# shamspias/fennec

Hardware: AMD Instinct MI355X
Metric: megapixels/sec: 4K SSIMFast+GaussianBlur (higher is better)
Workload: dtype u8 (blur: exact int32 sums of 24-bit fixed-point weights on the i8 matrix pipe; fp64 SSIM)

## Files before the change

fennec_amd/csrc/blur_mfma.hip:

```cpp
#include <hip/hip_ext.h>

#include "common.hpp"
#include "devutil.hpp"

#include <algorithm>
#include <cmath>
#include <type_traits>
#include <vector>

namespace fnx {

typedef int v4i __attribute__((ext_vector_type(4)));

constexpr int MF_RMAX = 6;
constexpr int MF_P = 48;
constexpr int MF_WT = 64 * MF_P + 256;
constexpr int MF_SP = 352;
constexpr int MF_OP = 272;
constexpr int MF_SEG_SCORE = 272;
constexpr int MF_SEG_SCORE_WIDE = 544;

struct MfmaArgs {
    const uint8_t *src;
    const uint8_t *const *srcs;
    uint8_t *dst;
    uint8_t *const *dsts;
    int sstride, dstride, w, h;
    int tiles_x, tiles, seg;
    int radius;
    const uint32_t *tab;
    int seed_h, seed_v, thr;
    const int32_t *bx, *by;
    const uint32_t *coltab, *rowtab;
    unsigned long long *slabs;
    int nbx, nby;
    int dbg;
    int narrow;
};

__device__ __forceinline__ int mf_comb3(int hi, int mid, int lo)
{
    int t = hi * 256 + mid;
    asm volatile("" : "+v"(t));
    return t * 256 + lo;
}

__device__ __forceinline__ const double *mf_scalar_ptr(const double *p)
{
    const unsigned long long v = reinterpret_cast<unsigned long long>(p);
    const unsigned lo = __builtin_amdgcn_readfirstlane(static_cast<unsigned>(v)), hi = __builtin_amdgcn_readfirstlane(static_cast<unsigned>(v >> 32));
    return reinterpret_cast<const double *>((static_cast<unsigned long long>(hi) << 32) | lo);
}
typedef __attribute__((address_space(1))) uint8_t mf_g_u8;
template <typename T> __device__ __forceinline__ T *mf_sgpr_ptr(T *p)
{
    unsigned long long v = reinterpret_cast<unsigned long long>(p);
    asm volatile("" : "+s"(v));
    return reinterpret_cast<T *>(v);
}
__device__ __forceinline__ void mf_lane_off(uint32_t &o) { asm volatile("" : "+v"(o)); }
typedef int mf_s16i __attribute__((ext_vector_type(16)));
__device__ __forceinline__ uint32_t mf_exact_u(const double *wd, const uint8_t *base, int step, int ring0, int mask)
{
    mf_s16i w0, w1;
    asm volatile("s_load_dwordx16 %0, %2, 0x0\n\ts_load_dwordx16 %1, %2, 0x40\n\ts_waitcnt lgkmcnt(0)" : "=&s"(w0), "=&s"(w1) : "s"(mf_scalar_ptr(wd)) : "memory");
    uint32_t v[13];
#pragma unroll
    for (int t = 0; t < 13; t++) v[t] = base[((ring0 + t) & mask) * step];
    double acc = 0;
#pragma unroll
    for (int t = 0; t < 13; t++) {
        const int lo = t < 8 ? w0[2 * (t & 7)] : w1[2 * (t & 7)], hi = t < 8 ? w0[2 * (t & 7) + 1] : w1[2 * (t & 7) + 1];
        acc = acc + u8_to_f64(v[t] ^ 0x80u) * __hiloint2double(hi, lo);
    }
    return clampF_dev(acc);
}

__device__ __forceinline__ void mf_box_add4(uint32_t *tbl, const u32x4 ro, uint32_t coln, const v4i cb)
{
#pragma unroll
    for (int k = 0; k < 4; k++)
        __hip_atomic_fetch_add(reinterpret_cast<uint32_t *>(reinterpret_cast<char *>(tbl) + ro[k] + coln), static_cast<uint32_t>(cb[k]),
                               __ATOMIC_RELAXED, __HIP_MEMORY_SCOPE_WORKGROUP);
}

template <bool SCORE, bool GUARD>
__global__ __launch_bounds__(256, GUARD ? 3 : 1) void blur_mfma_kernel(MfmaArgs a)
{
    constexpr int P = MF_P, WT = MF_WT, SP = MF_SP, OP = MF_OP;
    __shared__ __attribute__((aligned(16))) uint8_t s_t[4 * WT];
    __shared__ __attribute__((aligned(16))) uint8_t s_stage[2 * 16 * SP];
    __shared__ __attribute__((aligned(16))) uint8_t s_out[2 * 16 * OP];
    __shared__ __attribute__((aligned(16))) uint32_t s_rowh[SCORE ? MF_SEG_SCORE + 32 : 4];
    __shared__ __attribute__((aligned(16))) uint32_t s_rowv[SCORE ? MF_SEG_SCORE + 16 : 4];
    extern __shared__ __attribute__((aligned(16))) uint32_t s_box[];

    const int tile = xcd_tile(blockIdx.x, a.tiles);
    if (tile < 0) return;
    const int z = blockIdx.y;
    const uint8_t *src = a.srcs ? a.srcs[z] : a.src;
    uint8_t *dst = a.dsts ? a.dsts[z] : a.dst;
    const int ty = tile / a.tiles_x, tx = tile - ty * a.tiles_x;
    const int x0 = tx * 64, y0 = ty * a.seg;
    const int tid = threadIdx.x, wave = tid >> 6, lane = tid & 63;
    const int r = lane & 15, g = lane >> 4;
    const int NJ = min(a.seg, ((a.h - y0 + 15) >> 4) << 4) >> 4;
    const int NI = NJ + 1;
    const bool xedge = x0 - 6 < 0 || x0 + 70 > a.w;

    const v4i *tbh = reinterpret_cast<const v4i *>(a.tab);
    const long *tbv = reinterpret_cast<const long *>(a.tab + 3 * 64 * 4);
    const v4i bh2 = tbh[lane], bh1 = tbh[64 + lane], bh0 = tbh[128 + lane];
    const long bv2 = tbv[lane], bv1 = tbv[64 + lane], bv0 = tbv[128 + lane];
    const bool alane = (r & 3) == 3;
    const int seed_hl = alane ? (1 << 23) + 128 : a.seed_h;
    const v4i sh = {seed_hl, seed_hl, seed_hl, seed_hl}, sv = {a.seed_v, a.seed_v, a.seed_v, a.seed_v};
    const v4i zero = {0, 0, 0, 0};
    const uint32_t sel01 = alane ? 0x0c0c0400u : 0x0c0c0703u, sel23 = alane ? 0x04000c0cu : 0x07030c0cu;

    uint8_t *tw = s_t + wave * WT;
    const int id1 = min(256 + tid, 16 * 19 - 1);
    const int srow0 = tid / 19, sch0 = tid - 19 * srow0, srow1 = id1 / 19, sch1 = id1 - 19 * srow1;
    const bool two = tid < 48;
    const int st_w0 = srow0 * SP + 16 * sch0, st_w1 = srow1 * SP + 16 * sch1;
    const int st_r = r * SP + 64 * wave + 16 * g;
    uint8_t *t_w = tw + r * P + 4 * g;
    const int m4 = r >> 2, mi = r & 3;
    const uint8_t *t_r = tw + (16 * m4 + mi) * P + 64 * m4 + 8 * g;
    const uint8_t *t_ro = tw + (16 * m4 + mi) * P + 64 * m4 + ((8 * g + 16) & 31);
    const uint8_t *t_ae = tw + (16 * g + 3) * P + 64 * g + r + 6;
    const uint8_t *t_ao = tw + (16 * g + 3) * P + 64 * g + ((r + 22) & 31);
    const int o_w = r * OP + 64 * wave + 16 * g;
    const int orow = tid >> 4, och = tid & 15;
    const int o_r = orow * OP + 16 * och;
    const int xo = x0 + 4 * och;

    v4i bbox = {0, 0, 0, 0}, sbox = {0, 0, 0, 0};
    uint32_t coln = 0;
    const int slabn = SCORE ? (a.nbx + 1) * (a.nby + 1) : 0;
    uint32_t *tbl_s = s_box, *tbl_b = s_box + 4 * slabn;
    auto score_setup = [&]() {
        const uint32_t cw = a.coltab[256 * tx + tid];
        const int nrow = (2 * a.seg + 16) >> 2;
        const int nrh = (a.seg + 16) >> 2;
        const u32x4 rw = reinterpret_cast<const u32x4 *>(a.rowtab)[static_cast<size_t>(ty) * nrow + min(tid, nrow - 1)];
        if (!(a.dbg & 4)) for (int e = tid; e < 2 * slabn; e += 256) reinterpret_cast<u32x4 *>(s_box)[e] = (u32x4){0u, 0u, 0u, 0u};
        if (tid < nrh) reinterpret_cast<u32x4 *>(s_rowh)[tid] = rw;
        else if (tid < nrow) reinterpret_cast<u32x4 *>(s_rowv)[tid - nrh] = rw;
        coln = cw & 0xfffffu;
        const int seed = static_cast<int>((cw >> 20) & 31u) << 7;
        sbox = (v4i){seed, seed, seed, seed};
        const uint32_t sh = (cw >> 29) << 3;
#pragma unroll
        for (int e = 0; e < 4; e++) bbox[e] = static_cast<int>(((cw >> (25 + e)) & 1u) << sh);
    };

    const double *wd = reinterpret_cast<const double *>(a.tab + 3 * 64 * 4 + 3 * 64 * 2);

    auto stage_write = [&](const u32x4 (&d)[2], int buf) {
        uint8_t *sb = s_stage + buf * 16 * SP;
        *reinterpret_cast<u32x4 *>(sb + st_w0) = d[0] ^ 0x80808080u;
        if (two) *reinterpret_cast<u32x4 *>(sb + st_w1) = d[1] ^ 0x80808080u;
    };
    auto hset = [&](int s, int buf, int slot) {
        const uint8_t *sbuf = s_stage + buf * 16 * SP;
        const uint8_t *sb = sbuf + st_r;
        if constexpr (!GUARD && !SCORE) {
#pragma unroll
            for (int hf = 0; hf < 2; hf++) {
                v4i c2[2], c1[2], c0[2];
#pragma unroll
                for (int q2 = 0; q2 < 2; q2++) {
                    const v4i A = *reinterpret_cast<const v4i *>(sb + 16 * (2 * hf + q2));
                    c2[q2] = __builtin_amdgcn_mfma_i32_16x16x64_i8(A, bh2, zero, 0, 0, 0);
                    c1[q2] = __builtin_amdgcn_mfma_i32_16x16x64_i8(A, bh1, zero, 0, 0, 0);
                    c0[q2] = __builtin_amdgcn_mfma_i32_16x16x64_i8(A, bh0, sh, 0, 0, 0);
                }
#pragma unroll
                for (int q2 = 0; q2 < 2; q2++) {
                    const int qq = 2 * hf + q2;
                    v4i u;
#pragma unroll
                    for (int k = 0; k < 4; k++) u[k] = mf_comb3(c2[q2][k], c1[q2][k], c0[q2][k]);
                    const uint32_t t01 = __builtin_amdgcn_perm((uint32_t)u[1], (uint32_t)u[0], sel01);
                    const uint32_t t23 = __builtin_amdgcn_perm((uint32_t)u[3], (uint32_t)u[2], sel23);
                    *reinterpret_cast<uint32_t *>(t_w + (16 * qq) * P + 64 * qq + 16 * slot) = t01 | t23;
                }
                __builtin_amdgcn_sched_barrier(0);
            }
            return;
        }
        v4i c2[4], c1[4], c0[4];
#pragma unroll
        for (int qq = 0; qq < 4; qq++) {
            const v4i A = *reinterpret_cast<const v4i *>(sb + 16 * qq);
            c2[qq] = __builtin_amdgcn_mfma_i32_16x16x64_i8(A, bh2, zero, 0, 0, 0);
            c1[qq] = __builtin_amdgcn_mfma_i32_16x16x64_i8(A, bh1, zero, 0, 0, 0);
            c0[qq] = __builtin_amdgcn_mfma_i32_16x16x64_i8(A, bh0, sh, 0, 0, 0);
        }
        if constexpr (SCORE) {
            const u32x2 lo = *reinterpret_cast<const u32x2 *>(sb + 24), hi = *reinterpret_cast<const u32x2 *>(sb + 32);
            const v4i A = {(int)lo.x, (int)lo.y, (int)hi.x, (int)hi.y};
            const v4i cb = __builtin_amdgcn_mfma_i32_16x16x64_i8(A, bbox, sbox, 0, 0, 0);
            const u32x4 ro = *reinterpret_cast<const u32x4 *>(s_rowh + 16 * s + 4 * g);
            if (!(a.dbg & 1)) mf_box_add4(tbl_s, ro, coln, cb);
        }
        v4i u[4];
#pragma unroll
        for (int qq = 0; qq < 4; qq++)
#pragma unroll
            for (int k = 0; k < 4; k++) u[qq][k] = mf_comb3(c2[qq][k], c1[qq][k], c0[qq][k]);
#pragma unroll
        for (int qq = 0; qq < 4; qq++) {
            const uint32_t t01 = __builtin_amdgcn_perm((uint32_t)u[qq][1], (uint32_t)u[qq][0], sel01);
            const uint32_t t23 = __builtin_amdgcn_perm((uint32_t)u[qq][3], (uint32_t)u[qq][2], sel23);
            *reinterpret_cast<uint32_t *>(t_w + (16 * qq) * P + 64 * qq + 16 * slot) = t01 | t23;
        }
        if constexpr (GUARD) {
            uint32_t m[4];
#pragma unroll
            for (int qq = 0; qq < 4; qq++) {
                const uint32_t f0 = static_cast<uint32_t>(u[qq][0]) & 0x00ffffffu, f1 = static_cast<uint32_t>(u[qq][1]) & 0x00ffffffu;
                const uint32_t f2 = static_cast<uint32_t>(u[qq][2]) & 0x00ffffffu, f3 = static_cast<uint32_t>(u[qq][3]) & 0x00ffffffu;
                m[qq] = min(min(min(f0, f1), f2), f3);
            }
            const uint32_t mm = min(min(min(m[0], m[1]), m[2]), m[3]);
            if (__builtin_amdgcn_ballot_w64(mm < static_cast<uint32_t>(a.thr))) {
                uint32_t fl = 0;
#pragma unroll
                for (int qq = 0; qq < 4; qq++)
#pragma unroll
                    for (int k = 0; k < 4; k++) fl |= ((static_cast<uint32_t>(u[qq][k]) & 0x00ffffffu) < static_cast<uint32_t>(a.thr) ? 1u : 0u) << (4 * qq + k);
                unsigned long long todo = __builtin_amdgcn_ballot_w64(fl != 0);
                while (todo) {
                    const int L = __builtin_ctzll(todo);
                    todo &= todo - 1;
                    uint32_t flL = __builtin_amdgcn_readlane(fl, L);
                    const int rL = L & 15, gL = L >> 4;
                    while (flL) {
                        const int b = __builtin_ctz(flL), qq = b >> 2, k = b & 3;
                        flL &= flL - 1;
                        const uint32_t e = mf_exact_u(wd, sbuf + (4 * gL + k) * SP + 4 * (16 * wave + 4 * qq + (rL >> 2)) + (rL & 3), 4, 0, 0xffff) ^ 0x80u;
                        if (lane == L) *(t_w + (16 * qq) * P + 64 * qq + 16 * slot + k) = static_cast<uint8_t>(e);
                    }
                }
            }
        }
    };
    auto vset = [&](int j, int buf, auto oddt) {
        constexpr bool ODD = decltype(oddt)::value;
        long A[4];
        uint32_t al[4];
#pragma unroll
        for (int q = 0; q < 4; q++) A[q] = *reinterpret_cast<const long *>((ODD ? t_ro : t_r) + (4 * q) * P);
#pragma unroll
        for (int q = 0; q < 4; q++) al[q] = *((ODD ? t_ao : t_ae) + (4 * q) * P);
        int u[4][3];
        if constexpr (!GUARD && !SCORE) {
#pragma unroll
            for (int hf = 0; hf < 2; hf++) {
                v4i c2[2], c1[2], c0[2];
#pragma unroll
                for (int q2 = 0; q2 < 2; q2++) {
                    c2[q2] = __builtin_amdgcn_mfma_i32_16x16x32_i8(A[2 * hf + q2], bv2, zero, 0, 0, 0);
                    c1[q2] = __builtin_amdgcn_mfma_i32_16x16x32_i8(A[2 * hf + q2], bv1, zero, 0, 0, 0);
                    c0[q2] = __builtin_amdgcn_mfma_i32_16x16x32_i8(A[2 * hf + q2], bv0, sv, 0, 0, 0);
                }
#pragma unroll
                for (int q2 = 0; q2 < 2; q2++)
#pragma unroll
                    for (int i = 0; i < 3; i++) u[2 * hf + q2][i] = mf_comb3(c2[q2][i], c1[q2][i], c0[q2][i]);
                __builtin_amdgcn_sched_barrier(0);
            }
        } else {
            v4i c2[4], c1[4], c0[4];
#pragma unroll
            for (int q = 0; q < 4; q++) {
                c2[q] = __builtin_amdgcn_mfma_i32_16x16x32_i8(A[q], bv2, zero, 0, 0, 0);
                c1[q] = __builtin_amdgcn_mfma_i32_16x16x32_i8(A[q], bv1, zero, 0, 0, 0);
                c0[q] = __builtin_amdgcn_mfma_i32_16x16x32_i8(A[q], bv0, sv, 0, 0, 0);
            }
#pragma unroll
            for (int q = 0; q < 4; q++)
#pragma unroll
                for (int i = 0; i < 3; i++) u[q][i] = mf_comb3(c2[q][i], c1[q][i], c0[q][i]);
        }
        u32x4 o;
#pragma unroll
        for (int q = 0; q < 4; q++) {
            const uint32_t t01 = __builtin_amdgcn_perm((uint32_t)u[q][1], (uint32_t)u[q][0], 0x0c0c0703u);
            const uint32_t t23 = __builtin_amdgcn_perm(al[q], (uint32_t)u[q][2], 0x04030c0cu);
            o[q] = t01 | t23;
        }
        uint8_t *op = s_out + buf * 16 * OP + o_w;
        *reinterpret_cast<u32x4 *>(op) = o;
        if constexpr (GUARD) {
            uint32_t m[4];
#pragma unroll
            for (int q = 0; q < 4; q++)
                m[q] = min(min(static_cast<uint32_t>(u[q][0]) & 0x00ffffffu, static_cast<uint32_t>(u[q][1]) & 0x00ffffffu), static_cast<uint32_t>(u[q][2]) & 0x00ffffffu);
            const uint32_t mm = min(min(min(m[0], m[1]), m[2]), m[3]);
            if (__builtin_amdgcn_ballot_w64(mm < static_cast<uint32_t>(a.thr))) {
                uint32_t fl = 0;
#pragma unroll
                for (int q = 0; q < 4; q++)
#pragma unroll
                    for (int i = 0; i < 3; i++) fl |= ((static_cast<uint32_t>(u[q][i]) & 0x00ffffffu) < static_cast<uint32_t>(a.thr) ? 1u : 0u) << (4 * q + i);
                unsigned long long todo = __builtin_amdgcn_ballot_w64(fl != 0);
                while (todo) {
                    const int L = __builtin_ctzll(todo);
                    todo &= todo - 1;
                    uint32_t flL = __builtin_amdgcn_readlane(fl, L);
                    const int rL = L & 15, gL = L >> 4;
                    while (flL) {
                        const int b = __builtin_ctz(flL), q = b >> 2, i = b & 3;
                        flL &= flL - 1;
                        const uint32_t e = mf_exact_u(wd, tw + (16 * gL + 4 * q + i) * P + 64 * gL, 1, (ODD ? 16 : 0) + rL, 31);
                        if (lane == L) op[4 * q + i] = static_cast<uint8_t>(e);
                    }
                }
                if constexpr (SCORE) o = *reinterpret_cast<const u32x4 *>(op);
            }
        }
        if constexpr (SCORE) {
            const u32x4 os = o ^ 0x80808080u;
            const v4i A = {(int)os[0], (int)os[1], (int)os[2], (int)os[3]};
            const v4i cb = __builtin_amdgcn_mfma_i32_16x16x64_i8(A, bbox, sbox, 0, 0, 0);
            const u32x4 ro = *reinterpret_cast<const u32x4 *>(s_rowv + 16 * j + 4 * g);
            if (!(a.dbg & 1)) mf_box_add4(tbl_b, ro, coln, cb);
        }
    };

    auto march = [&](auto formt) {
        constexpr int FORM = decltype(formt)::value;
        constexpr bool XEDGE = FORM == 2, INNER = FORM == 0;
        const uint8_t *in_base = INNER ? src + static_cast<ptrdiff_t>(y0 - 6) * a.sstride + 4 * static_cast<ptrdiff_t>(x0 - 6) : src;
        uint8_t *out_base = INNER ? dst + static_cast<ptrdiff_t>(y0) * a.dstride + 4 * static_cast<ptrdiff_t>(x0) : dst;
        const uint32_t ss = static_cast<uint32_t>(a.sstride), ds = static_cast<uint32_t>(a.dstride);
        const uint32_t in_set = 16u * ss, out_set = 16u * ds;
        uint32_t in_l0 = static_cast<uint32_t>(srow0) * ss + 16u * sch0, in_l1 = static_cast<uint32_t>(srow1) * ss + 16u * sch1;
        uint32_t out_l = static_cast<uint32_t>(orow) * ds + 16u * och;
        auto hload = [&](int i, u32x4 (&d)[2]) {
            const int ys = y0 - 6 + 16 * i;
            if constexpr (INNER) {
                const mf_g_u8 *sb = (const mf_g_u8 *)mf_sgpr_ptr(in_base + static_cast<uint32_t>(i) * in_set);
                mf_lane_off(in_l0);
                mf_lane_off(in_l1);
                d[0] = *(g_u32x4 *)(sb + in_l0);
                d[1] = *(g_u32x4 *)(sb + in_l1);
            } else if constexpr (!XEDGE) {
                const uint8_t *sb = src + 4 * static_cast<ptrdiff_t>(x0 - 6);
                const int ya = clampi(ys + srow0, 0, a.h - 1), yb = clampi(ys + srow1, 0, a.h - 1);
                d[0] = *(g_u32x4 *)(sb + static_cast<ptrdiff_t>(ya) * a.sstride + 16 * sch0);
                d[1] = *(g_u32x4 *)(sb + static_cast<ptrdiff_t>(yb) * a.sstride + 16 * sch1);
            } else {
    #pragma unroll
                for (int k = 0; k < 2; k++) {
                    if (k == 1 && !two) break;
                    const int y = clampi(ys + (k ? srow1 : srow0), 0, a.h - 1);
                    const uint8_t *rowp = src + static_cast<size_t>(y) * a.sstride;
                    const int xc = x0 - 6 + 4 * (k ? sch1 : sch0);
    #pragma unroll
                    for (int e = 0; e < 4; e++) d[k][e] = ld_px(rowp, clampi(xc + e, 0, a.w - 1));
                }
            }
        };
        auto out_store = [&](int j, int buf) {
            const u32x4 o = *reinterpret_cast<const u32x4 *>(s_out + buf * 16 * OP + o_r);
            if constexpr (INNER) {
                mf_lane_off(out_l);
                *(g_u32x4w *)((mf_g_u8 *)mf_sgpr_ptr(out_base + static_cast<uint32_t>(j) * out_set) + out_l) = o;
                return;
            }
            const int y = y0 + 16 * j + orow;
            if (y < a.h) {
                uint8_t *dp = dst + static_cast<size_t>(y) * a.dstride + 4 * static_cast<size_t>(xo);
                if (!XEDGE || xo + 3 < a.w) *(g_u32x4w *)(dp) = o;
                else {
    #pragma unroll
                    for (int e = 0; e < 4; e++) if (xo + e < a.w) *(g_u32w *)(dp + 4 * e) = o[e];
                }
            }
        };
        u32x4 ra[2], rb[2];
        hload(0, ra);
        __builtin_amdgcn_sched_barrier(0);
        hload(min(1, NI - 1), rb);
        __builtin_amdgcn_sched_barrier(0);
        if constexpr (SCORE) score_setup();
        auto step = [&](int s, u32x4 (&d)[2], auto oddv) {
            constexpr int par = decltype(oddv)::value ? 0 : 1;
            if (s < NI) stage_write(d, par);
            if (XEDGE) { if (s + 2 < NI) hload(s + 2, d); } else hload(min(s + 2, NI - 1), d);
            if (s >= 3 && s - 3 < NJ) out_store(s - 3, par);
            __syncthreads();
            if (s < NI) hset(s, par, par);
            if (s >= 1 && s - 1 < NJ) vset(s - 1, par, oddv);
        };
    #pragma unroll 1
        for (int s = 0; s < NJ + 3; s += 2) {
            step(s, ra, std::true_type{});
            step(s + 1, rb, std::false_type{});
        }

    };
    const bool inner = !xedge && a.narrow && y0 >= 6 && y0 + 16 * NJ + 10 <= a.h;
    if (xedge) march(std::integral_constant<int, 2>{});
    else if (inner) march(std::integral_constant<int, 0>{});
    else march(std::integral_constant<int, 1>{});

    if (SCORE && !(a.dbg & 2)) {
        __syncthreads();
        unsigned long long *slab = a.slabs + (static_cast<size_t>(z) * a.tiles + tile) * 2 * slabn;
        for (int e = tid; e < 2 * slabn; e += 256) {
            const u32x4 v = *reinterpret_cast<const u32x4 *>(s_box + 4 * e);
            slab[e] = static_cast<unsigned long long>(v.x | (v.y << 16)) | (static_cast<unsigned long long>(v.z) << 32);
        }
    }
}

template <int NKH> struct MfWide {
    static constexpr int NKV = NKH <= 4 ? 1 : (NKH <= 7 ? 2 : 3);
    static constexpr int RFH = 8 * NKH - 2, RFV = 32 * NKV - 8;
    static constexpr int RF = RFH < RFV ? RFH : RFV;
    static constexpr int NC = 16 + RF / 2;
    static constexpr int NL = (16 * NC + 255) / 256;
    static constexpr int SP = 16 * NC + 48;
    static constexpr int NT = 2 * RF + 1;
    static constexpr int NS = 4 * NKV;
    static constexpr int RING = 16 * NS;
    static constexpr int P = RING + 16;
    static constexpr int WT = 64 * P + 256;
};

template <int NT>
__device__ __noinline__ uint32_t mf_exact_h_n(const uint8_t *p, const double *wd)
{
    double acc = 0;
#pragma unroll 15
    for (int t = 0; t < NT; t++) acc = acc + u8_to_f64(p[4 * t] ^ 0x80u) * wd[t];
    return clampF_dev(acc);
}
template <int NT, int RING = 64>
__device__ __noinline__ uint32_t mf_exact_v_n(const uint8_t *p, int ring0, const double *wd)
{
    double acc = 0;
#pragma unroll 15
    for (int t = 0; t < NT; t++) acc = acc + u8_to_f64(p[static_cast<unsigned>(ring0 + t) % static_cast<unsigned>(RING)] ^ 0x80u) * wd[t];
    return clampF_dev(acc);
}

template <int NT>
__device__ __forceinline__ uint32_t mf_exact_u_n(const double *wd, const uint8_t *base, int step, int ring0, int mask)
{
    double acc = 0;
#pragma unroll
    for (int t0 = 0; t0 < NT; t0 += 8) {
        mf_s16i w;
        asm volatile("s_load_dwordx16 %0, %1, %2\n\ts_waitcnt lgkmcnt(0)" : "=&s"(w) : "s"(mf_scalar_ptr(wd)), "n"(8 * t0) : "memory");
        uint32_t v[8];
#pragma unroll
        for (int t = 0; t < 8; t++) v[t] = base[((ring0 + t0 + min(t, NT - 1 - t0)) & mask) * step];
#pragma unroll
        for (int t = 0; t < 8; t++)
            if (t0 + t < NT) acc = acc + u8_to_f64(v[t] ^ 0x80u) * __hiloint2double(w[2 * t + 1], w[2 * t]);
    }
    return clampF_dev(acc);
}

template <int NKH, bool GUARD, bool SCORE = false>
__global__ __launch_bounds__(256, MfWide<NKH>::NKV == 3 ? 1 : 2) void blur_mfma_wide_kernel(MfmaArgs a)
{
    using C = MfWide<NKH>;
    constexpr int RF = C::RF, NC = C::NC, SP = C::SP, P = C::P, WT = C::WT, OP = MF_OP, NT = C::NT;
    constexpr int NKV = C::NKV, NS = C::NS, RING = C::RING, NL = C::NL;
    static_assert(!SCORE || (4 * RF) % 8 == 0, "the source-side A operand is read as two 8-byte halves");
    static_assert(!SCORE || NKV == 1, "the one-pass form is NKH = 2's");
    __shared__ __attribute__((aligned(16))) uint8_t s_t[4 * WT];
    __shared__ __attribute__((aligned(16))) uint8_t s_stage[2 * 16 * SP];
    __shared__ __attribute__((aligned(16))) uint8_t s_out[2 * 16 * OP];
    __shared__ __attribute__((aligned(16))) uint32_t s_rowh[SCORE ? MF_SEG_SCORE_WIDE + 48 : 4];
    __shared__ __attribute__((aligned(16))) uint32_t s_rowv[SCORE ? MF_SEG_SCORE_WIDE + 16 : 4];
    __shared__ uint32_t s_colbox[SCORE ? 64 : 1];
    extern __shared__ __attribute__((aligned(16))) uint32_t s_box[];

    const int tile = xcd_tile(blockIdx.x, a.tiles);
    if (tile < 0) return;
    const int z = blockIdx.y;
    const uint8_t *src = a.srcs ? a.srcs[z] : a.src;
    uint8_t *dst = a.dsts ? a.dsts[z] : a.dst;
    const int ty = tile / a.tiles_x, tx = tile - ty * a.tiles_x;
    const int x0 = tx * 64, y0 = ty * a.seg;
    const int tid = threadIdx.x, wave = tid >> 6, lane = tid & 63;
    const int r = lane & 15, g = lane >> 4;
    const int NJ = min(a.seg, ((a.h - y0 + 15) >> 4) << 4) >> 4;
    const int NI = NJ + NS - 1;
    const bool xedge = x0 - RF < 0 || x0 + 64 + RF > a.w;

    const v4i *tbh = reinterpret_cast<const v4i *>(a.tab);
    v4i bh[NKH][3];
#pragma unroll
    for (int kk = 0; kk < NKH; kk++)
#pragma unroll
        for (int l = 0; l < 3; l++) bh[kk][l] = tbh[(3 * kk + l) * 64 + lane];
    const v4i *tbv = tbh + 3 * NKH * 64;
    v4i bv[NKV][3];
#pragma unroll
    for (int c = 0; c < NKV; c++)
#pragma unroll
        for (int l = 0; l < 3; l++) bv[c][l] = tbv[(3 * c + l) * 64 + lane];
    const double *wd = reinterpret_cast<const double *>(tbv + 3 * NKV * 64);
    const bool alane = (r & 3) == 3;
    const int seed_hl = alane ? (1 << 23) + 128 : a.seed_h;
    const v4i sh = {seed_hl, seed_hl, seed_hl, seed_hl}, sv = {a.seed_v, a.seed_v, a.seed_v, a.seed_v};
    const v4i zero = {0, 0, 0, 0};
    const uint32_t sel01 = alane ? 0x0c0c0400u : 0x0c0c0703u, sel23 = alane ? 0x04000c0cu : 0x07030c0cu;

    uint8_t *tw = s_t + wave * WT;
    int srow[NL], sch[NL], st_w[NL];
    bool have[NL];
#pragma unroll
    for (int k = 0; k < NL; k++) {
        const int id = min(256 * k + tid, 16 * NC - 1);
        srow[k] = id / NC; sch[k] = id - NC * srow[k];
        st_w[k] = srow[k] * SP + 16 * sch[k];
        have[k] = 256 * k + tid < 16 * NC;
    }
    const int st_r = r * SP + 64 * wave + 16 * g;
    uint8_t *t_w = tw + r * P + 4 * g;
    const int m4 = r >> 2, mi = r & 3;
    const uint8_t *t_r = tw + (16 * m4 + mi) * P + 64 * m4;
    const uint8_t *t_a = tw + (16 * g + 3) * P + 64 * g;
    const int o_w = r * OP + 64 * wave + 16 * g;
    const int orow = tid >> 4, och = tid & 15;
    const int o_r = orow * OP + 16 * och;
    const int xo = x0 + 4 * och;

    v4i bbox = {0, 0, 0, 0}, sbox = {0, 0, 0, 0};
    uint32_t coln = 0;
    const int slabn = SCORE ? (a.nbx + 1) * (a.nby + 1) : 0;
    uint32_t *tbl_s = s_box, *tbl_b = s_box + 4 * slabn;
    auto score_setup = [&]() {
        for (int e = tid; e < 8 * slabn; e += 256) s_box[e] = 0;
        const int rowbytes = 16 * (a.nbx + 1);
        const int b0y = a.by[y0];
        for (int u = tid; u < 16 * NI; u += 256) {
            const int t = u - RF;
            const int v = (t >= 0 && t < a.seg && y0 + t < a.h) ? a.by[y0 + t] : -1;
            s_rowh[u] = rowbytes * ((v >= 0 && b0y >= 0) ? v - b0y : a.nby);
        }
        for (int t = tid; t < 16 * NJ; t += 256) {
            const int v = (t < a.seg && y0 + t < a.h) ? a.by[y0 + t] : -1;
            s_rowv[t] = rowbytes * ((v >= 0 && b0y >= 0) ? v - b0y : a.nby);
        }
        if (tid < 64) {
            const int b0x = a.bx[x0], v = x0 + tid < a.w ? a.bx[x0 + tid] : -1;
            s_colbox[tid] = (v >= 0 && b0x >= 0) ? v - b0x : 255u;
        }
        __syncthreads();
        uint32_t first = 255u;
        for (int i = 0; i < 16; i++) first = min(first, s_colbox[16 * wave + i]);
        const int slot = r / 3, ch = r - 3 * slot;
        int cnt = 0;
        for (int i = 0; i < 16; i++) cnt += (r < 15 && s_colbox[16 * wave + i] == first + slot) ? 1 : 0;
#pragma unroll
        for (int e = 0; e < 4; e++) {
            const bool in = r < 15 && first != 255u && s_colbox[16 * wave + 4 * g + e] == first + slot;
            bbox[e] = in ? (1 << (8 * ch)) : 0;
        }
        const int seed = 128 * cnt;
        sbox = (v4i){seed, seed, seed, seed};
        const uint32_t bc = (r < 15 && first != 255u && cnt > 0) ? first + slot : static_cast<uint32_t>(a.nbx);
        coln = 16u * bc + 4u * (r < 15 ? ch : 3);
    };

    auto stage_write = [&](const u32x4 (&d)[NL], int buf) {
        uint8_t *sb = s_stage + buf * 16 * SP;
        *reinterpret_cast<u32x4 *>(sb + st_w[0]) = d[0] ^ 0x80808080u;
#pragma unroll
        for (int k = 1; k < NL; k++)
            if (have[k]) *reinterpret_cast<u32x4 *>(sb + st_w[k]) = d[k] ^ 0x80808080u;
    };
    auto hset = [&](int s, int buf, int slot) {
        const uint8_t *sbuf = s_stage + buf * 16 * SP;
        const uint8_t *sb = sbuf + st_r;
        v4i c2[4], c1[4], c0[4];
#pragma unroll
        for (int qq = 0; qq < 4; qq++) { c2[qq] = zero; c1[qq] = zero; c0[qq] = sh; }
        if constexpr (SCORE) {
            const u32x2 lo = *reinterpret_cast<const u32x2 *>(sb + 4 * RF), hi = *reinterpret_cast<const u32x2 *>(sb + 4 * RF + 8);
            const v4i A = {(int)lo.x, (int)lo.y, (int)hi.x, (int)hi.y};
            const v4i cb = __builtin_amdgcn_mfma_i32_16x16x64_i8(A, bbox, sbox, 0, 0, 0);
            const u32x4 ro = *reinterpret_cast<const u32x4 *>(s_rowh + 16 * s + 4 * g);
#pragma unroll
            for (int k = 0; k < 4; k++)
                __hip_atomic_fetch_add(reinterpret_cast<uint32_t *>(reinterpret_cast<char *>(tbl_s) + ro[k] + coln), static_cast<uint32_t>(cb[k]),
                                       __ATOMIC_RELAXED, __HIP_MEMORY_SCOPE_WORKGROUP);
        }
#pragma unroll
        for (int kk = 0; kk < NKH; kk++)
#pragma unroll
            for (int qq = 0; qq < 4; qq++) {
                const v4i A = *reinterpret_cast<const v4i *>(sb + 16 * qq + 64 * kk);
                c2[qq] = __builtin_amdgcn_mfma_i32_16x16x64_i8(A, bh[kk][0], c2[qq], 0, 0, 0);
                c1[qq] = __builtin_amdgcn_mfma_i32_16x16x64_i8(A, bh[kk][1], c1[qq], 0, 0, 0);
                c0[qq] = __builtin_amdgcn_mfma_i32_16x16x64_i8(A, bh[kk][2], c0[qq], 0, 0, 0);
            }
        v4i u[4];
#pragma unroll
        for (int qq = 0; qq < 4; qq++)
#pragma unroll
            for (int k = 0; k < 4; k++) u[qq][k] = mf_comb3(c2[qq][k], c1[qq][k], c0[qq][k]);
#pragma unroll
        for (int qq = 0; qq < 4; qq++) {
            const uint32_t t01 = __builtin_amdgcn_perm((uint32_t)u[qq][1], (uint32_t)u[qq][0], sel01);
            const uint32_t t23 = __builtin_amdgcn_perm((uint32_t)u[qq][3], (uint32_t)u[qq][2], sel23);
            *reinterpret_cast<uint32_t *>(t_w + (16 * qq) * P + 64 * qq + 16 * slot) = t01 | t23;
        }
        if constexpr (GUARD) {
            uint32_t m[4];
#pragma unroll
// ... 498 lines not shown
```

Measured before the change: 417,500.

## Skew ring group offsets and transpose vertical MFMA batching to drop alpha pass

```diff
diff --git a/fennec_amd/csrc/blur_mfma.hip b/fennec_amd/csrc/blur_mfma.hip
--- a/fennec_amd/csrc/blur_mfma.hip
+++ b/fennec_amd/csrc/blur_mfma.hip
@@ -19,6 +19,9 @@
 constexpr int MF_OP = 272;
 constexpr int MF_SEG_SCORE = 272;
 constexpr int MF_SEG_SCORE_WIDE = 544;
+
+__host__ __device__ constexpr int mf_skew(int grp) { return 80 * grp; }
+static_assert(64 * MF_P + mf_skew(3) <= MF_WT, "the ring's last group ends inside the wave's ring");
 
 struct MfmaArgs {
     const uint8_t *src;
@@ -126,10 +129,10 @@
     const int st_r = r * SP + 64 * wave + 16 * g;
     uint8_t *t_w = tw + r * P + 4 * g;
     const int m4 = r >> 2, mi = r & 3;
-    const uint8_t *t_r = tw + (16 * m4 + mi) * P + 64 * m4 + 8 * g;
-    const uint8_t *t_ro = tw + (16 * m4 + mi) * P + 64 * m4 + ((8 * g + 16) & 31);
-    const uint8_t *t_ae = tw + (16 * g + 3) * P + 64 * g + r + 6;
-    const uint8_t *t_ao = tw + (16 * g + 3) * P + 64 * g + ((r + 22) & 31);
+    const uint8_t *t_r = tw + (16 * m4 + 4 * mi) * P + mf_skew(m4) + 8 * g;
+    const uint8_t *t_ro = tw + (16 * m4 + 4 * mi) * P + mf_skew(m4) + ((8 * g + 16) & 31);
+    const uint8_t *t_ae = tw + (16 * g + 3) * P + mf_skew(g) + r + 6;
+    const uint8_t *t_ao = tw + (16 * g + 3) * P + mf_skew(g) + ((r + 22) & 31);
     const int o_w = r * OP + 64 * wave + 16 * g;
     const int orow = tid >> 4, och = tid & 15;
     const int o_r = orow * OP + 16 * och;
@@ -184,7 +187,7 @@
                     for (int k = 0; k < 4; k++) u[k] = mf_comb3(c2[q2][k], c1[q2][k], c0[q2][k]);
                     const uint32_t t01 = __builtin_amdgcn_perm((uint32_t)u[1], (uint32_t)u[0], sel01);
                     const uint32_t t23 = __builtin_amdgcn_perm((uint32_t)u[3], (uint32_t)u[2], sel23);
-                    *reinterpret_cast<uint32_t *>(t_w + (16 * qq) * P + 64 * qq + 16 * slot) = t01 | t23;
+                    *reinterpret_cast<uint32_t *>(t_w + (16 * qq) * P + mf_skew(qq) + 16 * slot) = t01 | t23;
                 }
                 __builtin_amdgcn_sched_barrier(0);
             }
@@ -214,7 +217,7 @@
         for (int qq = 0; qq < 4; qq++) {
             const uint32_t t01 = __builtin_amdgcn_perm((uint32_t)u[qq][1], (uint32_t)u[qq][0], sel01);
             const uint32_t t23 = __builtin_amdgcn_perm((uint32_t)u[qq][3], (uint32_t)u[qq][2], sel23);
-            *reinterpret_cast<uint32_t *>(t_w + (16 * qq) * P + 64 * qq + 16 * slot) = t01 | t23;
+            *reinterpret_cast<uint32_t *>(t_w + (16 * qq) * P + mf_skew(qq) + 16 * slot) = t01 | t23;
         }
         if constexpr (GUARD) {
             uint32_t m[4];
@@ -241,7 +244,7 @@
                         const int b = __builtin_ctz(flL), qq = b >> 2, k = b & 3;
                         flL &= flL - 1;
                         const uint32_t e = mf_exact_u(wd, sbuf + (4 * gL + k) * SP + 4 * (16 * wave + 4 * qq + (rL >> 2)) + (rL & 3), 4, 0, 0xffff) ^ 0x80u;
-                        if (lane == L) *(t_w + (16 * qq) * P + 64 * qq + 16 * slot + k) = static_cast<uint8_t>(e);
+                        if (lane == L) *(t_w + (16 * qq) * P + mf_skew(qq) + 16 * slot + k) = static_cast<uint8_t>(e);
                     }
                 }
             }
@@ -249,63 +252,65 @@
     };
     auto vset = [&](int j, int buf, auto oddt) {
         constexpr bool ODD = decltype(oddt)::value;
-        long A[4];
+        long A[3];
         uint32_t al[4];
 #pragma unroll
-        for (int q = 0; q < 4; q++) A[q] = *reinterpret_cast<const long *>((ODD ? t_ro : t_r) + (4 * q) * P);
-#pragma unroll
-        for (int q = 0; q < 4; q++) al[q] = *((ODD ? t_ao : t_ae) + (4 * q) * P);
-        int u[4][3];
+        for (int q = 0; q < 3; q++) A[q] = *reinterpret_cast<const long *>((ODD ? t_ro : t_r) + q * P);
+#pragma unroll
+        for (int i = 0; i < 4; i++) al[i] = *((ODD ? t_ao : t_ae) + (4 * i) * P);
+        int u[3][4];
         if constexpr (!GUARD && !SCORE) {
 #pragma unroll
             for (int hf = 0; hf < 2; hf++) {
+                const int nq = 2 - hf;
                 v4i c2[2], c1[2], c0[2];
 #pragma unroll
-                for (int q2 = 0; q2 < 2; q2++) {
+                for (int q2 = 0; q2 < nq; q2++) {
                     c2[q2] = __builtin_amdgcn_mfma_i32_16x16x32_i8(A[2 * hf + q2], bv2, zero, 0, 0, 0);
                     c1[q2] = __builtin_amdgcn_mfma_i32_16x16x32_i8(A[2 * hf + q2], bv1, zero, 0, 0, 0);
                     c0[q2] = __builtin_amdgcn_mfma_i32_16x16x32_i8(A[2 * hf + q2], bv0, sv, 0, 0, 0);
                 }
 #pragma unroll
-                for (int q2 = 0; q2 < 2; q2++)
-#pragma unroll
-                    for (int i = 0; i < 3; i++) u[2 * hf + q2][i] = mf_comb3(c2[q2][i], c1[q2][i], c0[q2][i]);
+                for (int q2 = 0; q2 < nq; q2++)
+#pragma unroll
+                    for (int i = 0; i < 4; i++) u[2 * hf + q2][i] = mf_comb3(c2[q2][i], c1[q2][i], c0[q2][i]);
                 __builtin_amdgcn_sched_barrier(0);
             }
         } else {
-            v4i c2[4], c1[4], c0[4];
-#pragma unroll
-            for (int q = 0; q < 4; q++) {
+            v4i c2[3], c1[3], c0[3];
+#pragma unroll
+            for (int q = 0; q < 3; q++) {
                 c2[q] = __builtin_amdgcn_mfma_i32_16x16x32_i8(A[q], bv2, zero, 0, 0, 0);
                 c1[q] = __builtin_amdgcn_mfma_i32_16x16x32_i8(A[q], bv1, zero, 0, 0, 0);
                 c0[q] = __builtin_amdgcn_mfma_i32_16x16x32_i8(A[q], bv0, sv, 0, 0, 0);
             }
 #pragma unroll
-            for (int q = 0; q < 4; q++)
-#pragma unroll
-                for (int i = 0; i < 3; i++) u[q][i] = mf_comb3(c2[q][i], c1[q][i], c0[q][i]);
+            for (int q = 0; q < 3; q++)
+#pragma unroll
+                for (int i = 0; i < 4; i++) u[q][i] = mf_comb3(c2[q][i], c1[q][i], c0[q][i]);
         }
         u32x4 o;
 #pragma unroll
-        for (int q = 0; q < 4; q++) {
-            const uint32_t t01 = __builtin_amdgcn_perm((uint32_t)u[q][1], (uint32_t)u[q][0], 0x0c0c0703u);
-            const uint32_t t23 = __builtin_amdgcn_perm(al[q], (uint32_t)u[q][2], 0x04030c0cu);
-            o[q] = t01 | t23;
+        for (int i = 0; i < 4; i++) {
+            const uint32_t t01 = __builtin_amdgcn_perm((uint32_t)u[1][i], (uint32_t)u[0][i], 0x0c0c0703u);
+            const uint32_t t23 = __builtin_amdgcn_perm(al[i], (uint32_t)u[2][i], 0x04030c0cu);
+            o[i] = t01 | t23;
         }
         uint8_t *op = s_out + buf * 16 * OP + o_w;
         *reinterpret_cast<u32x4 *>(op) = o;
         if constexpr (GUARD) {
-            uint32_t m[4];
-#pragma unroll
-            for (int q = 0; q < 4; q++)
-                m[q] = min(min(static_cast<uint32_t>(u[q][0]) & 0x00ffffffu, static_cast<uint32_t>(u[q][1]) & 0x00ffffffu), static_cast<uint32_t>(u[q][2]) & 0x00ffffffu);
-            const uint32_t mm = min(min(min(m[0], m[1]), m[2]), m[3]);
+            uint32_t m[3];
+#pragma unroll
+            for (int q = 0; q < 3; q++)
+                m[q] = min(min(min(static_cast<uint32_t>(u[q][0]) & 0x00ffffffu, static_cast<uint32_t>(u[q][1]) & 0x00ffffffu),
+                               static_cast<uint32_t>(u[q][2]) & 0x00ffffffu), static_cast<uint32_t>(u[q][3]) & 0x00ffffffu);
+            const uint32_t mm = min(min(m[0], m[1]), m[2]);
             if (__builtin_amdgcn_ballot_w64(mm < static_cast<uint32_t>(a.thr))) {
                 uint32_t fl = 0;
 #pragma unroll
-                for (int q = 0; q < 4; q++)
-#pragma unroll
-                    for (int i = 0; i < 3; i++) fl |= ((static_cast<uint32_t>(u[q][i]) & 0x00ffffffu) < static_cast<uint32_t>(a.thr) ? 1u : 0u) << (4 * q + i);
+                for (int q = 0; q < 3; q++)
+#pragma unroll
+                    for (int i = 0; i < 4; i++) fl |= ((static_cast<uint32_t>(u[q][i]) & 0x00ffffffu) < static_cast<uint32_t>(a.thr) ? 1u : 0u) << (4 * q + i);
                 unsigned long long todo = __builtin_amdgcn_ballot_w64(fl != 0);
                 while (todo) {
                     const int L = __builtin_ctzll(todo);
@@ -315,8 +320,8 @@
                     while (flL) {
                         const int b = __builtin_ctz(flL), q = b >> 2, i = b & 3;
                         flL &= flL - 1;
-                        const uint32_t e = mf_exact_u(wd, tw + (16 * gL + 4 * q + i) * P + 64 * gL, 1, (ODD ? 16 : 0) + rL, 31);
-                        if (lane == L) op[4 * q + i] = static_cast<uint8_t>(e);
+                        const uint32_t e = mf_exact_u(wd, tw + (16 * gL + 4 * i + q) * P + mf_skew(gL), 1, (ODD ? 16 : 0) + rL, 31);
+                        if (lane == L) op[4 * i + q] = static_cast<uint8_t>(e);
                     }
                 }
                 if constexpr (SCORE) o = *reinterpret_cast<const u32x4 *>(op);
```

After: 428,000 (median of 6 runs). +2.5%, better.
